# JarryChou/qcrypto-ldpc

Hardware: AMD Instinct MI355X
Metric: reconciled_key_Mbit_s (higher is better)
Workload: dtype f32

## Files before the change

### qcrypto-ldpc_amd/csrc/qldpc_engine.hip

```cpp
#include <hip/hip_runtime.h>

#include <algorithm>
#include <chrono>
#include <cstdio>
#include <cstdlib>
#include <cstring>
#include <new>
#include <optional>
#include <type_traits>
#include <vector>

#include "qldpc_engine_int.h"
#include "qldpc_kernels_edge.h"
#include "qldpc_kernels_chain.h"
#include "qldpc_kernels_compact.h"
#include "qldpc_kernels_fpost.h"
#include "qldpc_kernels_weakest.h"

extern "C" int qldpc_device_count(void)
{
    int n = 0;
    if (hipGetDeviceCount(&n) != hipSuccess) return 0;
    return n;
}
// ... 380 lines not shown
                if (code->max_dv < 32768) {
                    if ((rc = dev_alloc(d, &d->d_chain_order, (size_t)d->M)) || (rc = dev_alloc(d, &d->d_chain_dep, (size_t)d->E)) ||
                        (rc = dev_alloc(d, &d->d_chain_ver, (size_t)d->G * d->N)) || (rc = dev_alloc(d, &d->d_chain_ctl, QC_CTL_WORDS))) return rc;
                    HIPCHK(hipMemcpy(d->d_chain_order, chain_order.data(), sizeof(int) * (size_t)d->M, hipMemcpyHostToDevice));
                    HIPCHK(hipMemcpy(d->d_chain_dep, depv.data(), sizeof(int) * (size_t)d->E, hipMemcpyHostToDevice));
                    d->chain = 1;
                }
            }
        }
    }
    const size_t G = (size_t)d->G, FG = (size_t)d->FG;
    if (cfg->schedule == QLDPC_SCHED_FLOODING) {
        const size_t elems = d->msg_i8 ? (G * d->E * FG + 3) / 4 : (d->msg_half ? (G * d->E * FG + 1) / 2 : G * d->E * FG);
        if (d->msg_i8 && (rc = dev_alloc(d, &d->d_llr8, G * d->N * 64))) return rc;
        const char *coded_env = getenv("QLDPC_CODED_LLR");
        if (!(coded_env && coded_env[0] == '0') && (!d->msg_i8 || (coded_env && coded_env[0] == '1'))) {
            if ((rc = dev_alloc(d, &d->d_ybits, G * d->N * V))) return rc;
            if ((rc = dev_alloc(d, &d->d_fmag, G * FG))) return rc;
            if ((rc = dev_alloc(d, &d->d_fnch, G * FG))) return rc;
            if ((rc = dev_alloc(d, &d->d_vcls, ((size_t)d->N + 3) / 4 * 4))) return rc;
        }
        if ((rc = dev_alloc(d, &d->d_a, elems))) return rc;
        if ((rc = dev_alloc(d, &d->d_b, elems))) return rc;
        {
            bool ok = !d->msg_i8 && !d->msg_half && d->V == 1 && family_of(cfg->rule) == QK_FAM_MS && !cfg->enable_syndrome && code->max_dc <= QK_FP_DCMAX;
            for (auto &b : d->cn_buckets) ok = ok && b.cap > 0;
            if (const char *e = getenv("QLDPC_FLOOD_POST")) ok = ok && atoi(e) != 0;
            std::vector<uint32_t> tab;
            if (ok) { tab.resize((size_t)d->M); ok = qldpc_code_chain_table(code, tab.data()) == 1; }
            if (ok) {
                d->ira_K = code->ira_K;
                d->fp_vn = 1;
                if (const char *e = getenv("QLDPC_FLOOD_POST_VN")) d->fp_vn = atoi(e) != 0;
                if ((rc = make_buckets(d, code->vn_ptr, nullptr, d->ira_K, VN_CAPS, 2, d->fp_vn_buckets))) return rc;
                if (d->fp_vn) {
                    std::vector<int> vt((size_t)d->E);
                    for (int k = 0; k < d->E; k++) vt[(size_t)code->transpose[k]] = k;
                    if ((rc = make_fp_vn_classes(d, code->vn_ptr, d->ira_K, vt.data(), d->fp_vn_classes))) return rc;
                }
                if ((rc = dev_alloc(d, &d->d_fp_chain, (size_t)d->M))) return rc;
                HIPCHK(hipMemcpy(d->d_fp_chain, tab.data(), sizeof(uint32_t) * (size_t)d->M, hipMemcpyHostToDevice));
                const size_t post_n = G * d->N * 64, st_n = G * d->M * (64 * QK_FP_ROWS);
                float *base = d->d_a;
                if (post_n + 2 * st_n > elems) { if ((rc = dev_alloc(d, &d->d_fp_mem, post_n + 2 * st_n))) return rc; base = d->d_fp_mem; }
                d->fp_post = base; d->fp_st[0] = base + post_n; d->fp_st[1] = base + post_n + st_n;
                d->fpost = 1;
            }
        }
    } else if (d->msg_i8) {
        if ((rc = dev_alloc(d, &d->d_llr8, G * d->N * 64))) return rc;
        if ((rc = dev_alloc(d, &d->d_a, G * d->N * 64))) return rc;
        if ((rc = dev_alloc(d, &d->d_b, G * d->E * 64))) return rc;
    } else {
        if ((rc = dev_alloc(d, &d->d_a, G * d->N * FG))) return rc;
        if ((rc = dev_alloc(d, &d->d_b, G * d->E * FG))) return rc;
    }
    if ((rc = dev_alloc(d, &d->d_sgn, G * d->N * V))) return rc;
    if (d->msg_i8) d->d_hard = d->d_sgn;
    else if ((rc = dev_alloc(d, &d->d_hard, G * d->N * V))) return rc;
    if ((rc = dev_alloc(d, &d->d_unsat, G * V))) return rc;
    if ((rc = dev_alloc(d, &d->d_done, G * V))) return rc;
    if ((rc = dev_alloc(d, &d->d_depth, G * FG))) return rc;
    if ((rc = dev_alloc(d, &d->d_iters, G * FG))) return rc;
    d->gu.patience = cfg->giveup_patience;
    if (d->gu.patience > 0 && ((rc = dev_alloc(d, &d->gu.weight, G * FG)) || (rc = dev_alloc(d, &d->gu.last, G * FG)) || (rc = dev_alloc(d, &d->gu.best, G * FG)) ||
                               (rc = dev_alloc(d, &d->gu.since, G * FG)) || (rc = dev_alloc(d, &d->gu.gave, G * V)) || (rc = dev_alloc(d, &d->gu.total, 1)))) return rc;
// ... 116 lines not shown
    if (!d) return QLDPC_EINVAL;
    HIPCHK(hipSetDevice(d->device));
    HIPCHK(hipStreamSynchronize(d->stream));
    return QLDPC_OK;
}


struct prof_scope {
    qldpc_decoder *d; int kind; double bytes, moved; hipEvent_t a, b; bool on;
    prof_scope(qldpc_decoder *d_, int kind_, double bytes_, double moved_ = -1.0) : d(d_), kind(kind_), bytes(bytes_), moved(moved_ < 0.0 ? bytes_ : moved_), a(nullptr), b(nullptr), on(d_->prof_on != 0)
    {
        if (on) { (void)hipEventCreate(&a); (void)hipEventCreate(&b); (void)hipEventRecord(a, d->stream); }
    }
    ~prof_scope()
    {
        if (on) { (void)hipEventRecord(b, d->stream); d->prof_pending.push_back({kind, bytes, moved, a, b}); }
    }
};

extern "C" int qldpc_profile_enable(qldpc_decoder *d, int on) { if (!d) return QLDPC_EINVAL; d->prof_on = on; return QLDPC_OK; }

static int prof_fold(qldpc_decoder *d)
{
    if (d->prof_pending.empty()) return QLDPC_OK;
    HIPCHK(hipStreamSynchronize(d->stream));
    for (auto &r : d->prof_pending) {
        float ms = 0.0f;
        if (hipEventElapsedTime(&ms, r.a, r.b) == hipSuccess) {
            d->stats[r.kind].launches++;
            d->stats[r.kind].total_ms += ms;
            d->stats[r.kind].alg_bytes += r.bytes;
            d->stats[r.kind].moved_bytes += r.moved;
        }
        (void)hipEventDestroy(r.a); (void)hipEventDestroy(r.b);
    }
    d->prof_pending.clear();
    return QLDPC_OK;
}

extern "C" int qldpc_profile_read(qldpc_decoder *d, qldpc_kernel_stat *out, int cap)
{
    if (!d || (!out && cap > 0)) return QLDPC_EINVAL;
    HIPCHK(hipSetDevice(d->device));
    int rc = prof_fold(d);
    if (rc) return rc;
    int n = 0;
    for (int k = 0; k < KS_COUNT && n < cap; k++) if (d->stats[k].launches) out[n++] = d->stats[k];
    return n;
}

extern "C" int qldpc_profile_clear(qldpc_decoder *d)
{
    if (!d) return QLDPC_EINVAL;
    int rc = prof_fold(d);
    if (rc) return rc;
    for (int k = 0; k < KS_COUNT; k++) { d->stats[k].launches = 0; d->stats[k].total_ms = 0; d->stats[k].alg_bytes = 0; d->stats[k].moved_bytes = 0; }
    return QLDPC_OK;
}


static double msg_b(const qldpc_decoder *d) { return d->msg_i8 ? 1.0 : (d->msg_half ? 2.0 : 4.0); }
static double llr_b(const qldpc_decoder *d) { return d->msg_i8 ? 1.0 : 4.0; }
static double live_frames(const qldpc_decoder *d) { return (double)(d->live_lanes > 0 && d->live_lanes < d->n_frames ? d->live_lanes : d->n_frames); }
static double bytes_cn(const qldpc_decoder *d) { return 2.0 * d->E * msg_b(d) * live_frames(d); }
static double bytes_vn(const qldpc_decoder *d, int mode)
{
    if (mode != QK_VN_NORMAL) return ((double)d->E * msg_b(d) + d->N * llr_b(d)) * live_frames(d);
    return (2.0 * d->E * msg_b(d) + d->N * llr_b(d)) * live_frames(d);
}
// ... 26 lines not shown
template <int V, int MODE>
static int vn_pass(qldpc_decoder *d, float *post_out)
{
    prof_scope ps(d, KS_VN, bytes_vn(d, MODE), moved_vn(d, MODE));
    for (auto &b : d->vn_buckets) { qldpc_launch_vn<V, MODE>(d, b, post_out); LAUNCHCHK(); }
    return QLDPC_OK;
}
template <int V>
static int cn_pass(qldpc_decoder *d, bool first = false)
{
    prof_scope ps(d, KS_CN, bytes_cn(d), first && !d->msg_i8 ? ((double)d->E * msg_b(d) + d->N / 8.0) * live_frames(d) : -1.0);
    for (auto &b : d->cn_buckets) { qldpc_launch_cn<V>(d, b, first); LAUNCHCHK(); }
    d->remap_src = nullptr;
    return QLDPC_OK;
}
static double fp_info_edges(const qldpc_decoder *d) { return (double)d->E - (2.0 * d->M - 1.0); }
static double fp_chan(const qldpc_decoder *d, double vns) { return d->llr_coded ? vns / 8.0 : vns * 4.0; }
static double moved_cn_fpost(const qldpc_decoder *d, bool first)
{
    const double Ei = fp_info_edges(d), st = (double)QK_FP_ROWS * d->M * 4.0;
    if (first) return (Ei * 4.0 + st + fp_chan(d, d->N)) * live_frames(d);
    return (2.0 * Ei * 4.0 + 2.0 * st + fp_chan(d, d->M)) * live_frames(d);
}
static double moved_vn_fpost(const qldpc_decoder *d, bool rows_out, bool ballots)
{
    return (fp_info_edges(d) * 4.0 + fp_chan(d, d->ira_K) + (rows_out ? d->ira_K * 4.0 : 0.0) + (ballots ? d->ira_K / 4.0 : 0.0)) * live_frames(d);
}
static double fp_vn_rec_bytes(const qldpc_decoder *d)
{
    double b = 0.0;
    for (auto &c : d->fp_vn_classes) b += (double)c.n * QK_FPV_STRIDE(c.deg) * 4.0;
    return b * (live_frames(d) / 64.0);
}
static int cn_pass_fpost(qldpc_decoder *d, int ite)
{
    prof_scope ps(d, KS_CN, bytes_cn(d), moved_cn_fpost(d, ite == 0));
    for (auto &b : d->cn_buckets) { qldpc_launch_cn_fpost(d, b, ite); LAUNCHCHK(); }
    d->fp_last = ite & 1;
    return QLDPC_OK;
}
static int vn_pass_fpost(qldpc_decoder *d, float *post_out, bool between)
{
    const bool own = between && d->fp_vn;
    prof_scope ps(d, KS_VN, bytes_vn(d, QK_VN_POST), moved_vn_fpost(d, post_out != nullptr, !between) + (own ? fp_vn_rec_bytes(d) : 0.0));
    d->fp_between = between ? 1 : 0;
    if (own) { qldpc_launch_vn_fpost(d); LAUNCHCHK(); }
    for (auto &b : d->fp_vn_buckets)
        if (!own || b.cap == 0) { qldpc_launch_vn<1, QK_VN_POST>(d, b, post_out); LAUNCHCHK(); }
    d->fp_between = 0;
    return QLDPC_OK;
}
static int close_fpost(qldpc_decoder *d, float *post_out)
{
    const double b = ((double)QK_FP_ROWS * d->M * 4.0 + fp_chan(d, d->M) + (post_out ? d->M * 4.0 : 0.0) + d->M / 4.0) * live_frames(d);
    prof_scope ps(d, KS_VN, b, b);
    qldpc_launch_fpost_close(d, post_out);
    LAUNCHCHK();
    return QLDPC_OK;
}
static int run_flooding_post(qldpc_decoder *d)
{
    int rc;
    const int n_ite = d->cfg.n_ite;
    for (int ite = 0; ite < n_ite; ite++) {
        if ((rc = cn_pass_fpost(d, ite))) return rc;
        if (ite < n_ite - 1 && (rc = vn_pass_fpost(d, d->fp_post, true))) return rc;
    }
    d->last_iters = n_ite;
    if ((rc = vn_pass_fpost(d, nullptr, false))) return rc;
    return close_fpost(d, nullptr);
}

template <int V>
static int synd_pass(qldpc_decoder *d, const u64 *mask, int skip_done)
{
    prof_scope ps(d, KS_SYND, (double)d->E * 8.0 * d->G * V);
    const int g8 = (d->G + 7) / 8 * 8;
    const int Mp = (skip_done && d->M >= 4096) ? ((d->M / 8 + 255) / 256) * 256 : d->M;
    for (int part = 0; part < (Mp < d->M ? 2 : 1); part++) {
        const int lo = part ? Mp : 0, hi = part ? d->M : Mp;
        const int bx = std::max(1, std::min((hi - lo + 255) / 256, 4096 / std::max(1, d->G)));
        hipLaunchKernelGGL((qk_syndrome<V>), dim3((unsigned)((d->G < 8 ? d->G : g8) * bx)), dim3(256), 0, d->stream, mask, d->d_cn_var_t, d->max_dc, d->M, d->N,
                           d->d_unsat, d->d_done, skip_done, target_synd(d), d->G, bx, lo, hi, part);
    }
    LAUNCHCHK();
    return QLDPC_OK;
}
template <int V>
static int status_pass(qldpc_decoder *d, int ite_done)
{
    prof_scope ps(d, KS_STATUS, 0.0);
    hipLaunchKernelGGL((qk_status<V>), dim3((unsigned)d->G), dim3(64), 0, d->stream, d->d_unsat, d->d_done, d->d_depth, d->d_iters, d->G,
                       d->cfg.syndrome_depth, ite_done, d->d_active, d->d_work, (volatile int *)d->h_active_dev, ++d->poll_seq);
    LAUNCHCHK();
    return QLDPC_OK;
}
// ... 1094 lines not shown
    HIPCHK(hipSetDevice(d->device));
    return for_each_gen(d, [&](const int *origin, const u64 *fin, int n_slots) -> int {
        dim3 gs((unsigned)((n_slots + 255) / 256));
        with_v(d, [&](auto v) { hipLaunchKernelGGL((qk_giveup_out<v()>), gs, dim3(256), 0, d->stream, d->gu, d_gave, d_last_weight, d_best_weight, n_slots, origin, fin); });
        LAUNCHCHK();
        return (int)QLDPC_OK;
    });
}

extern "C" int qldpc_giveup_total(qldpc_decoder *d, uint64_t *frames)
{
    if (!d || !frames) return QLDPC_EINVAL;
    *frames = 0;
    if (d->gu.patience <= 0) return QLDPC_OK;
    HIPCHK(hipSetDevice(d->device));
    unsigned long long n = 0;
    HIPCHK(hipMemcpyAsync(&n, d->gu.total, sizeof(n), hipMemcpyDeviceToHost, d->stream));
    HIPCHK(hipStreamSynchronize(d->stream));
    *frames = n;
    return QLDPC_OK;
}

static int post_rows(qldpc_decoder *d, const char *who, const float **rows)
{
    int rc;
    if (d->cur_gen != 0) {
        qldpc_set_error("%s: the run compacted its active frames (%d times), the messages of frames that converged earlier are gone; "
                        "create the decoder with compact = 2 (or freeze_messages = 1) to read posteriors", who, d->compactions);
        return QLDPC_EUNSUPPORTED;
    }
    const float *src;
    if (d->cfg.schedule == QLDPC_SCHED_FLOODING) {
        if (!d->d_post) { if ((rc = dev_alloc(d, &d->d_post, (size_t)d->G * d->N * d->FG))) return rc; }
        if (d->fpost) { if ((rc = vn_pass_fpost(d, d->d_post, false)) || (rc = close_fpost(d, d->d_post))) return rc; }
        else if ((rc = with_v(d, [&](auto v) { return vn_pass<v(), QK_VN_POST>(d, d->d_post); }))) return rc;
        src = d->d_post;
    } else if (d->msg_i8) {
        if (!d->d_post) { if ((rc = dev_alloc(d, &d->d_post, (size_t)d->G * d->N * d->FG))) return rc; }
        const size_t n_dwords = (size_t)d->G * d->N * 64;
        hipLaunchKernelGGL(qi_post_to_f32, dim3((unsigned)std::min<size_t>((n_dwords + 255) / 256, 16384)), dim3(256), 0, d->stream, (const uint32_t *)d->d_a, d->d_post, n_dwords);
        LAUNCHCHK();
        src = d->d_post;
    } else {
        src = d->d_a;
    }
    *rows = src;
    return QLDPC_OK;
}

extern "C" int qldpc_fetch_post_dev(qldpc_decoder *d, float *d_post_out)
{
    if (!d || !d_post_out) return QLDPC_EINVAL;
    int rc = need_ran(d, "qldpc_fetch_post_dev");
    if (rc) return rc;
    HIPCHK(hipSetDevice(d->device));
    if (d->engine == QLDPC_ENGINE_EDGES) {
        return edge_vn<QK_VN_POST>(d, 0, 0, 1, d_post_out, -1);
    }
    const float *src;
    if ((rc = post_rows(d, "qldpc_fetch_post_dev", &src))) return rc;
    dim3 grid((unsigned)((d->N + 63) / 64), (unsigned)d->G);
    with_v(d, [&](auto v) { hipLaunchKernelGGL((qk_unload_f32<v()>), grid, dim3(256), 0, d->stream, src, d_post_out, d->N, d->n_frames); });
    LAUNCHCHK();
    return QLDPC_OK;
}

extern "C" int qldpc_fetch_weakest_dev(qldpc_decoder *d, const uint32_t *d_cand_bits, const int *d_take, int n_weak, uint32_t *d_weak_bits)
// ... 43 lines not shown
```

### qcrypto-ldpc_amd/csrc/qldpc_engine_int.h

```cpp
#ifndef QLDPC_ENGINE_INT_H
#define QLDPC_ENGINE_INT_H

#include <hip/hip_runtime.h>

#include <algorithm>
#include <vector>

#include "qldpc_hip.h"
#include "qldpc_kernels.h"
#include "qldpc_kernels_i8.h"
#include "qldpc_kernels_gang.h"
#include "qldpc_kernels_giveup.h"

enum { KS_CN = 0, KS_VN, KS_LAYER, KS_SYND, KS_STATUS, KS_LOAD, KS_FETCH, KS_VLAYER, KS_LAYER_REMAP, KS_COMPACT_ROWS, KS_LAYER_GANG, KS_COUNT };
static const char *const ks_names[KS_COUNT] = {"cn_update", "vn_update", "layer_update", "syndrome", "status", "load", "fetch", "vn_vlayer", "layer_update_remap", "compact_rows", "layer_update_gang"};

struct prof_rec { int kind; double bytes, moved; hipEvent_t a, b; };

struct bucket { int cap; int n; int *d_list; int *d_rec; };

struct fp_vn_class { int deg; int n; int *d_rec; };

struct gen_state {
    int G, cap;
    u64 *sgn, *hard, *unsat, *done, *ybits, *synd, *ebits;
    int *depth, *iters, *origin, *src;
    float *fmag; int *fnch;
    float *llr; uint32_t *llr8;
    int *gu_last, *gu_best, *gu_since; u64 *gu_gave;
    float *post, *msg;
};
#define QLDPC_MAX_GENS 6

struct qldpc_decoder {
    qldpc_decoder_cfg cfg;
    int N, M, E, K;
    int V, FG, G;
    int device;
    hipStream_t stream;
    int *d_cn_ptr, *d_cn_tr, *d_cn_var, *d_vn_ptr, *d_info_pos;
    int *d_vn_tr;
    int *d_cn_var_t, max_dc;
    std::vector<bucket> cn_buckets, vn_buckets;
    std::vector<std::vector<bucket>> layer_buckets;
    int n_layers;
    std::vector<bucket> vlayer_classes;
    int *d_vn_chk;
    double vl_rows;
    int layer_cst;
    int chain, chain_blocks, chain_lds; int *d_chain_order, *d_chain_dep, *d_chain_ver, *d_chain_ctl;
    qk_gang_entry *d_gang; std::vector<int> gang_off;
    int fpost, ira_K;
    std::vector<bucket> fp_vn_buckets;
    std::vector<fp_vn_class> fp_vn_classes;
    uint32_t *d_fp_chain;
    float *fp_post, *fp_st[2];
    float *d_fp_mem;
    int fp_last;
    int fp_between;
    int fp_vn;
    int layer_first;
    float *d_llr, *d_a, *d_b;
    float *d_post;
    u64 *d_sgn, *d_hard, *d_unsat, *d_done;
    int *d_depth, *d_iters, *d_active;
    int *h_active, *h_active_dev;
    int poll_seq;
    unsigned long long *d_work;
    qk_giveup gu;
    int G0;
    std::vector<gen_state> gens;
    int cur_gen, compact_mode, compactions;
    int live_lanes;
    float compact_ratio;
    const int *remap_src;
    const float *remap_msg;
    int *d_gcount, *d_goff;
    int llr_alt_cap[2]; float *d_llr_alt[2]; uint32_t *d_llr8_alt[2];
    int lay_alt_cap[2]; float *d_post_alt[2], *d_msg_alt[2];
    size_t bytes;
    int n_frames;
    int loaded, ran;
    int last_iters;
    int poll_every;
    u64 *d_synd;
    uint32_t *e_synd;
    int has_synd;
    float *h_in; int *h_out;
    int msg_half;
    u64 *d_ybits; float *d_fmag; int *d_fnch; uint8_t *d_vcls; int llr_coded;
    u64 *d_ebits; int has_erase;
    uint32_t *d_known; int has_known;
    int post_closes_run;
// ... 52 lines not shown
{
    if (mode == QK_VN_POST && d->fp_between) return 0;
    if (mode == QK_VN_POST) return 1 | (d->post_closes_run ? 2 : 0);
    return d->cfg.enable_syndrome ? 1 : 0;
}

struct gang_slot { int member, entry, n; };
struct gang_class { int cap, fam, cst; std::vector<gang_slot> slots; };
typedef std::vector<std::vector<gang_class>> gang_steps;
static inline void gang_plan_add(gang_steps &steps, int step, int cap, int fam, int cst, gang_slot s)
{
    if ((int)steps.size() <= step) steps.resize((size_t)step + 1);
    for (auto &c : steps[(size_t)step])
        if (c.cap == cap && c.fam == fam && c.cst == cst) { c.slots.push_back(s); return; }
    steps[(size_t)step].push_back(gang_class{cap, fam, cst, {s}});
}
struct qldpc_gang {
    std::vector<qldpc_decoder *> m;
    gang_steps steps;
    std::vector<int> buckets;
    int device;
    hipStream_t stream;
    long long stats[4];
};
int qldpc_launch_layer_gang(hipStream_t stream, int cap, int fam, int cst, const qk_gang_args &a, unsigned grid);

template <int V> void qldpc_launch_cn(qldpc_decoder *d, const bucket &b, bool first);
template <int V> void qldpc_launch_layer(qldpc_decoder *d, const bucket &b);
template <int V> void qldpc_launch_vlayer(qldpc_decoder *d, const bucket &b);
void qldpc_launch_layer_chain(qldpc_decoder *d, int sweep);
void qldpc_launch_cn_fpost(qldpc_decoder *d, const bucket &b, int ite);
void qldpc_launch_fpost_close(qldpc_decoder *d, float *post_out);
void qldpc_launch_vn_fpost(qldpc_decoder *d);
int qldpc_chain_resident_blocks(qldpc_decoder *d);
template <int V, int MODE> void qldpc_launch_vn(qldpc_decoder *d, const bucket &b, float *post_out);
#define QLDPC_DECLARE_LAUNCH(V)                                                                   \
    extern template void qldpc_launch_cn<V>(qldpc_decoder *, const bucket &, bool);                \
    extern template void qldpc_launch_layer<V>(qldpc_decoder *, const bucket &);                   \
    extern template void qldpc_launch_vlayer<V>(qldpc_decoder *, const bucket &);                  \
    extern template void qldpc_launch_vn<V, QK_VN_FIRST>(qldpc_decoder *, const bucket &, float *); \
    extern template void qldpc_launch_vn<V, QK_VN_NORMAL>(qldpc_decoder *, const bucket &, float *); \
    extern template void qldpc_launch_vn<V, QK_VN_POST>(qldpc_decoder *, const bucket &, float *);

#endif
```

### qcrypto-ldpc_amd/csrc/qldpc_kernels.h

```cpp
#ifndef QLDPC_KERNELS_H
#define QLDPC_KERNELS_H

#include <hip/hip_runtime.h>
#include <hip/hip_fp16.h>
#include <stdint.h>

typedef unsigned long long u64;

#ifndef QK_WAVES
#define QK_WAVES 4
#endif
#define QK_THREADS (QK_WAVES * 64)
#define QK_IDX_PAD 64

#define QK_FAM_MS 0
#define QK_REC_HDR 4
#define QK_FAM_SPA 1
#define QK_FAM_LSPA 2
#define QK_FAM_AMS 3

struct qk_rule {
    int rule;
    float param;
};
// ... 420 lines not shown
                for (int j = 0; j < V; j++) x[j] = qk_first_v2c(x[j], vin);
            } else if constexpr (REMAP) {
#pragma unroll
                for (int j = 0; j < V; j++) x[j] = qk_ldm1(vin_r[j] + (size_t)cn_tr[b + k] * FG);
            } else qk_load<V>(x, vin + (size_t)cn_tr[b + k] * FG);
#pragma unroll
            for (int j = 0; j < V; j++) qk_acc_in<FAM>(acc[j], qk_prep<FAM>(x[j]), rule);
        }
#pragma unroll
        for (int j = 0; j < V; j++) acc[j].finish(rule);
        for (int k = 0; k < deg; k++) {
            float x[V], o[V];
            const size_t off = (size_t)cn_tr[b + k] * FG;
            if constexpr (FIRST) {
                qk_coded_y<V>(x, coded, g, cn_var[b + k], N, lane, mg, nc);
#pragma unroll
                for (int j = 0; j < V; j++) x[j] = qk_first_v2c(x[j], vin);
            } else if constexpr (REMAP) {
#pragma unroll
                for (int j = 0; j < V; j++) x[j] = qk_ldm1(vin_r[j] + off);
            } else qk_load<V>(x, vin + off);
#pragma unroll
            for (int j = 0; j < V; j++) o[j] = acc[j].out(qk_prep<FAM>(x[j]), rule);
            qk_store_masked<V>(cout + (size_t)(b + k) * FG, o, frozen, any_frozen);
        }
    }
}


#define QK_VN_FIRST 0
#define QK_VN_NORMAL 1
#define QK_VN_POST 2

template <int V, int DVMAX, int UN, int MODE, typename MT, bool CODED = false>
__global__ __launch_bounds__(QK_THREADS) void qk_vn_flood(const MT *__restrict__ c2v, const float *__restrict__ llr,
                                                          MT *__restrict__ v2c, u64 *__restrict__ sgn, u64 *__restrict__ hard,
                                                          float *__restrict__ post_out,
                                                          const int *__restrict__ list, int n_list,
                                                          const int *__restrict__ vn_ptr, int N, size_t group_stride,
                                                          const u64 *__restrict__ done, qk_coded_llr coded = qk_coded_llr{}, int want_ballots = 1,
                                                          const int *__restrict__ vn_tr = nullptr)
{
    constexpr int FG = 64 * V;
    const int g = blockIdx.y;
    if ((MODE != QK_VN_POST || (want_ballots & 2)) && qk_group_done<V>(done, g)) return;
    const int lane = threadIdx.x & 63;
    const int wave = __builtin_amdgcn_readfirstlane(threadIdx.x >> 6);
    const MT *cin = c2v + (size_t)g * group_stride + lane * V;
    MT *vout = v2c + (size_t)g * group_stride + lane * V;
    const float *yin = llr + (size_t)g * N * FG + lane * V;
    const int i0 = (blockIdx.x * QK_WAVES + wave) * UN;
    if (i0 >= n_list) return;

    int vv[UN], bb[UN], dd[UN];
#pragma unroll
    for (int u = 0; u < UN; u++) {
        const int i = (i0 + u < n_list) ? i0 + u : i0;
        vv[u] = list[i];
    }
#pragma unroll
    for (int u = 0; u < UN; u++) { bb[u] = vn_ptr[vv[u]]; dd[u] = vn_ptr[vv[u] + 1] - bb[u]; }
    float y[UN][V], tmp[UN][V];
    auto channel = [&]() {
        if constexpr (CODED) {
            float mg[V];
            int nc[V];
#pragma unroll
            for (int j = 0; j < V; j++) { mg[j] = coded.fmag[(size_t)g * FG + lane * V + j]; nc[j] = coded.fnch[(size_t)g * FG + lane * V + j]; }
#pragma unroll
            for (int u = 0; u < UN; u++) qk_coded_y<V>(y[u], coded, g, vv[u], N, lane, mg, nc);
        } else {
#pragma unroll
            for (int u = 0; u < UN; u++) qk_ldm<V>(y[u], yin + (size_t)vv[u] * FG);
        }
    };
    if constexpr (MODE == QK_VN_FIRST || DVMAX <= 0) channel();

    if constexpr (MODE == QK_VN_FIRST) {
#pragma unroll
        for (int u = 0; u < UN; u++) {
            float o[V];
#pragma unroll
            for (int j = 0; j < V; j++) { tmp[u][j] = y[u][j] + 0.0f; o[j] = tmp[u][j] - 0.0f; }
            for (int k = 0; k < dd[u]; k++) qk_stm<V>(vout + (size_t)(bb[u] + k) * FG, o);
        }
    } else if constexpr (DVMAX > 0) {
        int tr[UN][DVMAX];
#pragma unroll
        for (int u = 0; u < UN; u++) {
#pragma unroll
            for (int k = 0; k < DVMAX; k++) tr[u][k] = vn_tr[bb[u] + k];
        }
        float m[UN][DVMAX][V];
#pragma unroll
        for (int u = 0; u < UN; u++) {
#pragma unroll
            for (int k = 0; k < DVMAX; k++)
                if (k < dd[u]) qk_ldm<V>(m[u][k], cin + (size_t)tr[u][k] * FG);
        }
        channel();
#pragma unroll
        for (int u = 0; u < UN; u++) {
            float sum[V];
#pragma unroll
            for (int j = 0; j < V; j++) sum[j] = 0.0f;
#pragma unroll
            for (int k = 0; k < DVMAX; k++)
                if (k < dd[u]) {
#pragma unroll
                    for (int j = 0; j < V; j++) sum[j] += m[u][k][j];
                }
#pragma unroll
            for (int j = 0; j < V; j++) tmp[u][j] = y[u][j] + sum[j];
            if constexpr (MODE == QK_VN_NORMAL) {
#pragma unroll
                for (int k = 0; k < DVMAX; k++)
                    if (k < dd[u]) {
                        float o[V];
#pragma unroll
                        for (int j = 0; j < V; j++) o[j] = tmp[u][j] - m[u][k][j];
                        qk_stm<V>(vout + (size_t)(bb[u] + k) * FG, o);
                    }
            }
        }
    } else {
#pragma unroll
        for (int u = 0; u < UN; u++) {
            float sum[V];
#pragma unroll
            for (int j = 0; j < V; j++) sum[j] = 0.0f;
            for (int k = 0; k < dd[u]; k++) {
                float m[V];
                qk_load<V>(m, cin + (size_t)vn_tr[bb[u] + k] * FG);
// ... 591 lines not shown
```

### qcrypto-ldpc_amd/csrc/qldpc_kernels_fpost.h

```cpp
#ifndef QLDPC_KERNELS_FPOST_H
#define QLDPC_KERNELS_FPOST_H

#include "qldpc_kernels.h"

#define QK_FP_ROWS 3
#define QK_FP_DCMAX 27
#define QK_FP_NONE 0xffu

__device__ __forceinline__ float qk_fp_msg(uint32_t w, int k, float c1, float c2)
{
    return qk_withsign(((int)(w >> 27) == k) ? c1 : c2, (w >> k) << 31);
}

template <int DCMAX, bool FIRST, bool CODED>
__global__ __launch_bounds__(QK_THREADS) void qk_cn_fpost(const float *__restrict__ post, const float *__restrict__ llr, float *__restrict__ c2v,
                                                          const float *st_in, float *st_out,
                                                          const int *__restrict__ list, int n_list,
                                                          const int *__restrict__ cn_ptr, const int *__restrict__ cn_var, const uint32_t *__restrict__ chain,
                                                          size_t group_stride, const u64 *__restrict__ done, qk_rule rule, const u64 *__restrict__ synd, int M, int N,
                                                          qk_coded_llr coded)
{
    static_assert(DCMAX > 0 && DCMAX <= QK_FP_DCMAX, "sign bits and the index share one word");
    const int g = blockIdx.y;
    const int lane = threadIdx.x & 63;
// ... 71 lines not shown
    }
    {
        const float own = qk_fp_msg(w, rp, c1, c2);
        const float sum0 = 0.0f + own;
        const float sum = (rnb != (int)QK_FP_NONE) ? sum0 + qk_fp_msg(rw, rnb & 31, rc1, rc2) : sum0;
        const float tmp = yr + sum;
        xr = tmp - own;
    }
    qk_acc<QK_FAM_MS> acc;
    acc.begin();
    if (synd) acc.sign = (uint32_t)((synd[(size_t)g * M + c] >> lane) & 1ull) << 31;
#pragma unroll
    for (int k = 0; k < DCMAX; k++)
        if (k < deg) {
            if (k == lpos) x[k] = xl;
            if (k == rpos) x[k] = xr;
            acc.in(x[k]);
        }
    acc.finish(rule);
    float *cout = c2v + (size_t)g * group_stride + lane;
    uint32_t nw = 0u, idx = 0u;
#pragma unroll
    for (int k = 0; k < DCMAX; k++)
        if (k < deg) {
            const float o = acc.out(x[k], rule);
            if (k != lpos && k != rpos) __builtin_nontemporal_store(o, cout + (size_t)(b + k) * 64);
            nw |= (qk_bits(o) >> 31) << k;
        }
#pragma unroll
    for (int k = DCMAX - 1; k >= 0; k--)
        if (k < deg) idx = (fabsf(x[k]) == acc.min1) ? (uint32_t)k : idx;
    float *so = st_out + srow;
    so[0] = acc.cst1; so[64] = acc.cst2; reinterpret_cast<uint32_t *>(so)[128] = nw | (idx << 27);
}

#define QK_FPV_DMAX 12
#define QK_FPV_CLASSES 4
#define QK_FPV_STRIDE(D) (((D) + 1 + 3) & ~3)
#define QK_FPV_UN(D) ((D) <= 4 ? 4 : 2)
struct qk_fpv_args {
    const int *rec[QK_FPV_CLASSES];
    int n[QK_FPV_CLASSES], deg[QK_FPV_CLASSES], blk_end[QK_FPV_CLASSES];
};
template <int D, int UN, bool CODED>
__device__ __forceinline__ void qk_vn_fpost_deg(const float *__restrict__ cin, const float *__restrict__ yin, float *__restrict__ pout,
                                                const int *__restrict__ rec, int n_list, int i0, int g, int lane, int N,
                                                const u64 *__restrict__ done, const qk_coded_llr &coded)
{
    constexpr int S = QK_FPV_STRIDE(D);
    if (i0 >= n_list) return;
    int w[UN][S];
#pragma unroll
    for (int u = 0; u < UN; u++) {
        const int i = (i0 + u < n_list) ? i0 + u : i0;
        const int4 *r = reinterpret_cast<const int4 *>(rec) + (size_t)i * (S / 4);
#pragma unroll
        for (int q = 0; q < S / 4; q++) {
            const int4 t = r[q];
            w[u][4 * q] = t.x; w[u][4 * q + 1] = t.y; w[u][4 * q + 2] = t.z; w[u][4 * q + 3] = t.w;
        }
    }
    if (qk_group_done<1>(done, g)) return;
    float m[UN][D > 0 ? D : 1];
#pragma unroll
    for (int u = 0; u < UN; u++) {
#pragma unroll
// ... 93 lines not shown
```

### qcrypto-ldpc_amd/csrc/qldpc_launch.hip

```cpp
#include "qldpc_engine_int.h"
#include "qldpc_kernels_h16.h"
#include "qldpc_kernels_cst.h"
#include "qldpc_kernels_vl.h"

#ifndef QL_V
#error "compile with -DQL_V=1, 2 or 4"
#endif

template <int V, int CAP, int FAM>
static void launch_cn_one(qldpc_decoder *d, const bucket &b, bool first)
{
    dim3 grid((unsigned)grid_x(b.n, 1), (unsigned)d->G);
    const qk_rule r = rule_of(d);
    if (first && !d->msg_i8) {
        const qk_coded_llr c = coded_llr_of(d);
        if (d->msg_half)
            hipLaunchKernelGGL((qk_cn_flood<V, CAP, FAM, __half, true>), grid, dim3(QK_THREADS), 0, d->stream, (const __half *)d->d_a, (__half *)d->d_b, b.d_list, b.n,
                               d->d_cn_ptr, d->d_cn_tr, (size_t)d->E * d->FG, d->d_done, r, d->freeze, target_synd(d), d->M, d->d_cn_var, d->N, c);
        else
            hipLaunchKernelGGL((qk_cn_flood<V, CAP, FAM, float, true>), grid, dim3(QK_THREADS), 0, d->stream, (const float *)d->d_a, d->d_b, b.d_list, b.n,
                               d->d_cn_ptr, d->d_cn_tr, (size_t)d->E * d->FG, d->d_done, r, d->freeze, target_synd(d), d->M, d->d_cn_var, d->N, c);
        return;
    }
    if (d->remap_src) {
// ... 153 lines not shown
                const qk_coded_llr c = coded_llr_of(d);
                hipLaunchKernelGGL((qi_vn_flood<CAP, UN, MODE, true>), grid, dim3(QK_THREADS), 0, d->stream, (const uint32_t *)d->d_b, (const uint32_t *)nullptr, (uint32_t *)d->d_a, d->d_sgn, (u64 *)nullptr,
                                   post_out, b.d_list, b.n, d->d_vn_ptr, d->N, (size_t)d->E * 64, d->d_done, c, d->quant_scale, want_ballots(d, MODE), d->d_vn_tr);
            } else
                hipLaunchKernelGGL((qi_vn_flood<CAP, UN, MODE, false>), grid, dim3(QK_THREADS), 0, d->stream, (const uint32_t *)d->d_b, d->d_llr8, (uint32_t *)d->d_a, d->d_sgn, (u64 *)nullptr,
                                   post_out, b.d_list, b.n, d->d_vn_ptr, d->N, (size_t)d->E * 64, d->d_done, qk_coded_llr{}, 0.0f, want_ballots(d, MODE), d->d_vn_tr);
        }
        return;
    }
    if (d->msg_half) launch_vn_k<V, CAP, UN, MODE, __half>(d, b, post_out);
    else launch_vn_k<V, CAP, UN, MODE, float>(d, b, post_out);
}
template <int V, int MODE>
void qldpc_launch_vn(qldpc_decoder *d, const bucket &b, float *post_out)
{
    if (MODE == QK_VN_FIRST) { launch_vn_one<V, 0, MODE>(d, b, post_out); return; }
    switch (b.cap) {
    case 4: launch_vn_one<V, 4, MODE>(d, b, post_out); break;
    case 12: launch_vn_one<V, 12, MODE>(d, b, post_out); break;
    default: launch_vn_one<V, 0, MODE>(d, b, post_out); break;
    }
}

template void qldpc_launch_cn<QL_V>(qldpc_decoder *, const bucket &, bool);
template void qldpc_launch_layer<QL_V>(qldpc_decoder *, const bucket &);
template void qldpc_launch_vlayer<QL_V>(qldpc_decoder *, const bucket &);
template void qldpc_launch_vn<QL_V, QK_VN_FIRST>(qldpc_decoder *, const bucket &, float *);
template void qldpc_launch_vn<QL_V, QK_VN_NORMAL>(qldpc_decoder *, const bucket &, float *);
template void qldpc_launch_vn<QL_V, QK_VN_POST>(qldpc_decoder *, const bucket &, float *);

#if QL_V == 1
#include "qldpc_kernels_fpost.h"

template <int DCMAX, bool FIRST>
static void launch_cn_fpost_one(qldpc_decoder *d, const bucket &b, int ite)
{
    dim3 grid((unsigned)grid_x(b.n, 1), (unsigned)d->G);
    const float *st_in = d->fp_st[(ite & 1) ^ 1];
    float *st_out = d->fp_st[ite & 1];
    if (d->llr_coded)
        hipLaunchKernelGGL((qk_cn_fpost<DCMAX, FIRST, true>), grid, dim3(QK_THREADS), 0, d->stream, (const float *)d->fp_post, (const float *)nullptr, d->d_b, st_in, st_out, b.d_list, b.n,
                           d->d_cn_ptr, d->d_cn_var, d->d_fp_chain, (size_t)d->E * 64, d->d_done, rule_of(d), target_synd(d), d->M, d->N, coded_llr_of(d));
    else
        hipLaunchKernelGGL((qk_cn_fpost<DCMAX, FIRST, false>), grid, dim3(QK_THREADS), 0, d->stream, (const float *)d->fp_post, (const float *)d->d_llr, d->d_b, st_in, st_out, b.d_list, b.n,
                           d->d_cn_ptr, d->d_cn_var, d->d_fp_chain, (size_t)d->E * 64, d->d_done, rule_of(d), target_synd(d), d->M, d->N, qk_coded_llr{});
}
void qldpc_launch_cn_fpost(qldpc_decoder *d, const bucket &b, int ite)
{
    switch (b.cap) {
    case 8: ite == 0 ? launch_cn_fpost_one<8, true>(d, b, ite) : launch_cn_fpost_one<8, false>(d, b, ite); break;
    case 12: ite == 0 ? launch_cn_fpost_one<12, true>(d, b, ite) : launch_cn_fpost_one<12, false>(d, b, ite); break;
    case 20: ite == 0 ? launch_cn_fpost_one<20, true>(d, b, ite) : launch_cn_fpost_one<20, false>(d, b, ite); break;
    default: ite == 0 ? launch_cn_fpost_one<QK_FP_DCMAX, true>(d, b, ite) : launch_cn_fpost_one<QK_FP_DCMAX, false>(d, b, ite); break;
    }
}
void qldpc_launch_vn_fpost(qldpc_decoder *d)
{
    const size_t nc = d->fp_vn_classes.size();
    for (size_t c0 = 0; c0 < nc; c0 += QK_FPV_CLASSES) {
        qk_fpv_args a{};
        int blocks = 0;
        for (size_t k = 0; k < QK_FPV_CLASSES; k++) {
            if (c0 + k < nc) {
                const fp_vn_class &c = d->fp_vn_classes[c0 + k];
                a.rec[k] = c.d_rec; a.n[k] = c.n; a.deg[k] = c.deg;
                blocks += grid_x(c.n, QK_FPV_UN(c.deg));
            }
            a.blk_end[k] = blocks;
        }
        dim3 grid((unsigned)blocks, (unsigned)d->G);
        if (d->llr_coded)
            hipLaunchKernelGGL((qk_vn_fpost<true>), grid, dim3(QK_THREADS), 0, d->stream, (const float *)d->d_b, (const float *)nullptr, d->fp_post, a,
                               d->N, (size_t)d->E * 64, d->d_done, coded_llr_of(d));
        else
            hipLaunchKernelGGL((qk_vn_fpost<false>), grid, dim3(QK_THREADS), 0, d->stream, (const float *)d->d_b, (const float *)d->d_llr, d->fp_post, a,
                               d->N, (size_t)d->E * 64, d->d_done, qk_coded_llr{});
    }
}
void qldpc_launch_fpost_close(qldpc_decoder *d, float *post_out)
{
    dim3 grid((unsigned)grid_x(d->M, 1), (unsigned)d->G);
    if (d->llr_coded)
        hipLaunchKernelGGL((qk_fpost_close<true>), grid, dim3(QK_THREADS), 0, d->stream, (const float *)d->fp_st[d->fp_last], (const float *)nullptr, d->d_fp_chain, d->d_sgn, d->d_hard, post_out,
                           d->M, d->N, d->ira_K, d->d_done, coded_llr_of(d));
    else
        hipLaunchKernelGGL((qk_fpost_close<false>), grid, dim3(QK_THREADS), 0, d->stream, (const float *)d->fp_st[d->fp_last], (const float *)d->d_llr, d->d_fp_chain, d->d_sgn, d->d_hard, post_out,
                           d->M, d->N, d->ira_K, d->d_done, qk_coded_llr{});
}

#include "qldpc_kernels_chain.h"

template <int DCMAX, int FAM>
static void launch_chain_one(qldpc_decoder *d, int sweep)
{
    const qk_rule r = rule_of(d);
    const int total = d->M * d->G;
    const unsigned grid = (unsigned)std::max(1, std::min((total + QK_WAVES - 1) / QK_WAVES, d->chain_blocks));
    hipLaunchKernelGGL((qk_cn_layer_chain<DCMAX, FAM>), dim3(grid), dim3(QK_THREADS), (size_t)d->chain_lds, d->stream, d->d_a, d->d_b, d->d_chain_order, d->M, d->G, d->d_cn_ptr, d->d_cn_var,
                       d->d_chain_dep, d->d_chain_ver, d->d_chain_ctl, sweep, d->N, (size_t)d->E * d->FG, d->d_done, r,
                       target_synd(d), d->layer_first, getenv("QLDPC_DEBUG") ? 1 : 0);
}
template <int FAM>
static void launch_chain_fam(qldpc_decoder *d, int sweep)
{
    if (d->max_dc <= 12) launch_chain_one<12, FAM>(d, sweep);
    else if (d->max_dc <= 20) launch_chain_one<20, FAM>(d, sweep);
    else launch_chain_one<40, FAM>(d, sweep);
}
void qldpc_launch_layer_chain(qldpc_decoder *d, int sweep)
{
    switch (family_of(d->cfg.rule)) {
    case QK_FAM_MS: launch_chain_fam<QK_FAM_MS>(d, sweep); break;
    case QK_FAM_SPA: launch_chain_fam<QK_FAM_SPA>(d, sweep); break;
    case QK_FAM_LSPA: launch_chain_fam<QK_FAM_LSPA>(d, sweep); break;
    default: launch_chain_fam<QK_FAM_AMS>(d, sweep); break;
    }
}
int qldpc_chain_resident_blocks(qldpc_decoder *d)
{
    int per_cu = 0, cus = 0;
// ... 14 lines not shown
```

Before: 2126.

## Batch groups in first flood-post CN pass and add scheduled final VN kernel

Adds a first-iteration check-node kernel that handles two to four frame groups per block. The code-structure loads (list, cn_ptr, cn_var, chain) are shared across those groups instead of being repeated per group. The final VN pass for degree-4 buckets now uses a variant with vectorised list loads and scheduling barriers that push memory loads ahead of use. Profiling scopes for the flood-post path are also reworked so consecutive kernels reuse a seam event instead of creating and recording two events each. The grouped kernel has fewer blocks and more registers per wave, which may reduce occupancy.

```diff
diff --git a/qcrypto-ldpc_amd/csrc/qldpc_engine.hip b/qcrypto-ldpc_amd/csrc/qldpc_engine.hip
--- a/qcrypto-ldpc_amd/csrc/qldpc_engine.hip
+++ b/qcrypto-ldpc_amd/csrc/qldpc_engine.hip
@@ -436,6 +436,12 @@
                 d->ira_K = code->ira_K;
                 d->fp_vn = 1;
                 if (const char *e = getenv("QLDPC_FLOOD_POST_VN")) d->fp_vn = atoi(e) != 0;
+                d->fp_first_groups = 4;
+                if (const char *e = getenv("QLDPC_FLOOD_POST_FIRST_GROUPS")) { const int x = atoi(e); if (x == 1 || x == 2 || x == 4) d->fp_first_groups = x; }
+                d->fp_close = 1;
+                if (const char *e = getenv("QLDPC_FLOOD_POST_CLOSE")) d->fp_close = atoi(e) != 0;
+                d->prof_markers = 0;
+                if (const char *e = getenv("QLDPC_PROF_MARKERS")) d->prof_markers = atoi(e) != 0;
                 if ((rc = make_buckets(d, code->vn_ptr, nullptr, d->ira_K, VN_CAPS, 2, d->fp_vn_buckets))) return rc;
                 if (d->fp_vn) {
                     std::vector<int> vt((size_t)d->E);
@@ -618,9 +624,10 @@
             d->stats[r.kind].alg_bytes += r.bytes;
             d->stats[r.kind].moved_bytes += r.moved;
         }
-        (void)hipEventDestroy(r.a); (void)hipEventDestroy(r.b);
-    }
+    }
+    for (auto &r : d->prof_pending) { if (!r.keep_a) (void)hipEventDestroy(r.a); (void)hipEventDestroy(r.b); }
     d->prof_pending.clear();
+    d->fp_seam = nullptr;
     return QLDPC_OK;
 }
 
@@ -713,9 +720,26 @@
     for (auto &c : d->fp_vn_classes) b += (double)c.n * QK_FPV_STRIDE(c.deg) * 4.0;
     return b * (live_frames(d) / 64.0);
 }
+struct fp_scope {
+    qldpc_decoder *d; int kind; double bytes, moved; hipEvent_t a; bool on, keep_a;
+    fp_scope(qldpc_decoder *d_, int kind_, double bytes_, double moved_) : d(d_), kind(kind_), bytes(bytes_), moved(moved_), a(nullptr), on(d_->prof_on != 0), keep_a(false)
+    {
+        if (!on) return;
+        if (!d->prof_markers && d->fp_seam) { a = d->fp_seam; keep_a = true; return; }
+        (void)hipEventCreate(&a); (void)hipEventRecord(a, d->stream);
+    }
+    ~fp_scope()
+    {
+        if (!on) return;
+        hipEvent_t b = nullptr;
+        (void)hipEventCreate(&b); (void)hipEventRecord(b, d->stream);
+        d->fp_seam = b;
+        d->prof_pending.push_back({kind, bytes, moved, a, b, keep_a});
+    }
+};
 static int cn_pass_fpost(qldpc_decoder *d, int ite)
 {
-    prof_scope ps(d, KS_CN, bytes_cn(d), moved_cn_fpost(d, ite == 0));
+    fp_scope ps(d, KS_CN, bytes_cn(d), moved_cn_fpost(d, ite == 0));
     for (auto &b : d->cn_buckets) { qldpc_launch_cn_fpost(d, b, ite); LAUNCHCHK(); }
     d->fp_last = ite & 1;
     return QLDPC_OK;
@@ -723,18 +747,22 @@
 static int vn_pass_fpost(qldpc_decoder *d, float *post_out, bool between)
 {
     const bool own = between && d->fp_vn;
-    prof_scope ps(d, KS_VN, bytes_vn(d, QK_VN_POST), moved_vn_fpost(d, post_out != nullptr, !between) + (own ? fp_vn_rec_bytes(d) : 0.0));
+    fp_scope ps(d, KS_VN, bytes_vn(d, QK_VN_POST), moved_vn_fpost(d, post_out != nullptr, !between) + (own ? fp_vn_rec_bytes(d) : 0.0));
     d->fp_between = between ? 1 : 0;
     if (own) { qldpc_launch_vn_fpost(d); LAUNCHCHK(); }
     for (auto &b : d->fp_vn_buckets)
-        if (!own || b.cap == 0) { qldpc_launch_vn<1, QK_VN_POST>(d, b, post_out); LAUNCHCHK(); }
+        if (!own || b.cap == 0) {
+            if (!between && b.cap == 4 && d->fp_close) qldpc_launch_vn_fpost_last(d, b, post_out);
+            else qldpc_launch_vn<1, QK_VN_POST>(d, b, post_out);
+            LAUNCHCHK();
+        }
     d->fp_between = 0;
     return QLDPC_OK;
 }
 static int close_fpost(qldpc_decoder *d, float *post_out)
 {
     const double b = ((double)QK_FP_ROWS * d->M * 4.0 + fp_chan(d, d->M) + (post_out ? d->M * 4.0 : 0.0) + d->M / 4.0) * live_frames(d);
-    prof_scope ps(d, KS_VN, b, b);
+    fp_scope ps(d, KS_VN, b, b);
     qldpc_launch_fpost_close(d, post_out);
     LAUNCHCHK();
     return QLDPC_OK;
@@ -743,6 +771,7 @@
 {
     int rc;
     const int n_ite = d->cfg.n_ite;
+    d->fp_seam = nullptr;
     for (int ite = 0; ite < n_ite; ite++) {
         if ((rc = cn_pass_fpost(d, ite))) return rc;
         if (ite < n_ite - 1 && (rc = vn_pass_fpost(d, d->fp_post, true))) return rc;
@@ -1903,7 +1932,7 @@
     const float *src;
     if (d->cfg.schedule == QLDPC_SCHED_FLOODING) {
         if (!d->d_post) { if ((rc = dev_alloc(d, &d->d_post, (size_t)d->G * d->N * d->FG))) return rc; }
-        if (d->fpost) { if ((rc = vn_pass_fpost(d, d->d_post, false)) || (rc = close_fpost(d, d->d_post))) return rc; }
+        if (d->fpost) { d->fp_seam = nullptr; if ((rc = vn_pass_fpost(d, d->d_post, false)) || (rc = close_fpost(d, d->d_post))) return rc; }
         else if ((rc = with_v(d, [&](auto v) { return vn_pass<v(), QK_VN_POST>(d, d->d_post); }))) return rc;
         src = d->d_post;
     } else if (d->msg_i8) {
diff --git a/qcrypto-ldpc_amd/csrc/qldpc_engine_int.h b/qcrypto-ldpc_amd/csrc/qldpc_engine_int.h
--- a/qcrypto-ldpc_amd/csrc/qldpc_engine_int.h
+++ b/qcrypto-ldpc_amd/csrc/qldpc_engine_int.h
@@ -15,7 +15,7 @@
 enum { KS_CN = 0, KS_VN, KS_LAYER, KS_SYND, KS_STATUS, KS_LOAD, KS_FETCH, KS_VLAYER, KS_LAYER_REMAP, KS_COMPACT_ROWS, KS_LAYER_GANG, KS_COUNT };
 static const char *const ks_names[KS_COUNT] = {"cn_update", "vn_update", "layer_update", "syndrome", "status", "load", "fetch", "vn_vlayer", "layer_update_remap", "compact_rows", "layer_update_gang"};
 
-struct prof_rec { int kind; double bytes, moved; hipEvent_t a, b; };
+struct prof_rec { int kind; double bytes, moved; hipEvent_t a, b; bool keep_a; };
 
 struct bucket { int cap; int n; int *d_list; int *d_rec; };
 
@@ -59,6 +59,10 @@
     int fp_last;
     int fp_between;
     int fp_vn;
+    int fp_first_groups;
+    int fp_close;
+    int prof_markers;
+    hipEvent_t fp_seam;
     int layer_first;
     float *d_llr, *d_a, *d_b;
     float *d_post;
@@ -177,6 +181,7 @@
 void qldpc_launch_cn_fpost(qldpc_decoder *d, const bucket &b, int ite);
 void qldpc_launch_fpost_close(qldpc_decoder *d, float *post_out);
 void qldpc_launch_vn_fpost(qldpc_decoder *d);
+void qldpc_launch_vn_fpost_last(qldpc_decoder *d, const bucket &b, float *post_out);
 int qldpc_chain_resident_blocks(qldpc_decoder *d);
 template <int V, int MODE> void qldpc_launch_vn(qldpc_decoder *d, const bucket &b, float *post_out);
 #define QLDPC_DECLARE_LAUNCH(V)                                                                   \
diff --git a/qcrypto-ldpc_amd/csrc/qldpc_kernels.h b/qcrypto-ldpc_amd/csrc/qldpc_kernels.h
--- a/qcrypto-ldpc_amd/csrc/qldpc_kernels.h
+++ b/qcrypto-ldpc_amd/csrc/qldpc_kernels.h
@@ -476,7 +476,7 @@
 #define QK_VN_NORMAL 1
 #define QK_VN_POST 2
 
-template <int V, int DVMAX, int UN, int MODE, typename MT, bool CODED = false>
+template <int V, int DVMAX, int UN, int MODE, typename MT, bool CODED = false, bool AHEAD = false>
 __global__ __launch_bounds__(QK_THREADS) void qk_vn_flood(const MT *__restrict__ c2v, const float *__restrict__ llr,
                                                           MT *__restrict__ v2c, u64 *__restrict__ sgn, u64 *__restrict__ hard,
                                                           float *__restrict__ post_out,
@@ -497,13 +497,29 @@
     if (i0 >= n_list) return;
 
     int vv[UN], bb[UN], dd[UN];
-#pragma unroll
-    for (int u = 0; u < UN; u++) {
-        const int i = (i0 + u < n_list) ? i0 + u : i0;
-        vv[u] = list[i];
-    }
-#pragma unroll
-    for (int u = 0; u < UN; u++) { bb[u] = vn_ptr[vv[u]]; dd[u] = vn_ptr[vv[u] + 1] - bb[u]; }
+    bool whole = false;
+    if constexpr (AHEAD) {
+        typedef int qk_ivec __attribute__((ext_vector_type(UN)));
+        whole = i0 + UN <= n_list;
+        if (whole) {
+            const qk_ivec t = *reinterpret_cast<const qk_ivec *>(list + i0);
+#pragma unroll
+            for (int u = 0; u < UN; u++) vv[u] = t[u];
+        }
+    }
+    if (!whole) {
+#pragma unroll
+        for (int u = 0; u < UN; u++) {
+            const int i = (i0 + u < n_list) ? i0 + u : i0;
+            vv[u] = list[i];
+        }
+    }
+    if constexpr (AHEAD) __builtin_amdgcn_sched_barrier(0);
+#pragma unroll
+    for (int u = 0; u < UN; u++) { bb[u] = vn_ptr[vv[u]]; dd[u] = vn_ptr[vv[u] + 1]; }
+    if constexpr (AHEAD) __builtin_amdgcn_sched_barrier(0);
+#pragma unroll
+    for (int u = 0; u < UN; u++) dd[u] -= bb[u];
     float y[UN][V], tmp[UN][V];
     auto channel = [&]() {
         if constexpr (CODED) {
@@ -535,6 +551,13 @@
 #pragma unroll
             for (int k = 0; k < DVMAX; k++) tr[u][k] = vn_tr[bb[u] + k];
         }
+        if constexpr (AHEAD) {
+#pragma unroll
+            for (int u = 0; u < UN; u++) {
+#pragma unroll
+                for (int k = 0; k < DVMAX; k++) asm volatile("" ::"s"(tr[u][k]));
+            }
+        }
         float m[UN][DVMAX][V];
 #pragma unroll
         for (int u = 0; u < UN; u++) {
@@ -543,6 +566,16 @@
                 if (k < dd[u]) qk_ldm<V>(m[u][k], cin + (size_t)tr[u][k] * FG);
         }
         channel();
+        if constexpr (AHEAD) {
+#pragma unroll
+            for (int u = 0; u < UN; u++) {
+#pragma unroll
+                for (int k = 0; k < DVMAX; k++) {
+#pragma unroll
+                    for (int j = 0; j < V; j++) asm volatile("" : "+v"(m[u][k][j]));
+                }
+            }
+        }
 #pragma unroll
         for (int u = 0; u < UN; u++) {
             float sum[V];
diff --git a/qcrypto-ldpc_amd/csrc/qldpc_kernels_fpost.h b/qcrypto-ldpc_amd/csrc/qldpc_kernels_fpost.h
--- a/qcrypto-ldpc_amd/csrc/qldpc_kernels_fpost.h
+++ b/qcrypto-ldpc_amd/csrc/qldpc_kernels_fpost.h
@@ -127,6 +127,102 @@
         if (k < deg) idx = (fabsf(x[k]) == acc.min1) ? (uint32_t)k : idx;
     float *so = st_out + srow;
     so[0] = acc.cst1; so[64] = acc.cst2; reinterpret_cast<uint32_t *>(so)[128] = nw | (idx << 27);
+}
+
+template <int DCMAX, bool CODED, int GW>
+__global__ __launch_bounds__(QK_THREADS) void qk_cn_fpost_first(const float *__restrict__ llr, float *__restrict__ c2v, float *__restrict__ st_out,
+                                                                const int *__restrict__ list, int n_list,
+                                                                const int *__restrict__ cn_ptr, const int *__restrict__ cn_var, const uint32_t *__restrict__ chain,
+                                                                size_t group_stride, const u64 *__restrict__ done, qk_rule rule, const u64 *__restrict__ synd, int M, int N, int G,
+                                                                qk_coded_llr coded)
+{
+    static_assert(DCMAX > 0 && DCMAX <= QK_FP_DCMAX, "sign bits and the index share one word");
+    static_assert(GW > 1 && GW <= 4, "a run of two to four groups");
+    const int g0 = blockIdx.y * GW;
+    const int lane = threadIdx.x & 63;
+    const int wave = __builtin_amdgcn_readfirstlane(threadIdx.x >> 6);
+    const int i = blockIdx.x * QK_WAVES + wave;
+    if (i >= n_list) return;
+    int gg[GW];
+    float mg[GW];
+    int nc[GW];
+    u64 dn[GW], sy[GW];
+#pragma unroll
+    for (int j = 0; j < GW; j++) {
+        gg[j] = (g0 + j < G) ? g0 + j : G - 1;
+        mg[j] = 0.0f; nc[j] = 0;
+        if constexpr (CODED) { mg[j] = coded.fmag[(size_t)gg[j] * 64 + lane]; nc[j] = coded.fnch[(size_t)gg[j] * 64 + lane]; }
+        dn[j] = done[gg[j]];
+    }
+    const int c = list[i];
+    const int b = cn_ptr[c];
+    const int deg = cn_ptr[c + 1] - b;
+    const uint32_t ch = chain[c];
+    const int lpos = (int)(ch & 0xffu), rpos = (int)((ch >> 8) & 0xffu);
+#pragma unroll
+    for (int j = 0; j < GW; j++) sy[j] = synd ? synd[(size_t)gg[j] * M + c] : 0ull;
+    int vid[DCMAX];
+    qk_coded_w wl[GW];
+    float y[CODED ? 1 : GW][DCMAX];
+    if constexpr (CODED) {
+        const int kl = lane < deg ? lane : (deg > 0 ? deg - 1 : 0);
+        const int vlane = cn_var[b + kl];
+        const uint32_t cls = (reinterpret_cast<const uint32_t *>(coded.vcls)[vlane >> 2] >> ((vlane & 3) * 8)) & 0xffu;
+        const u64 *eb = coded.ebits ? coded.ebits : coded.ybits;
+        const u64 em = coded.ebits ? ~0ull : 0ull;
+#pragma unroll
+        for (int j = 0; j < GW; j++) {
+            const size_t at = (size_t)gg[j] * N + vlane;
+            wl[j].cls = cls; wl[j].yb = coded.ybits[at]; wl[j].eb = eb[at] & em;
+        }
+#pragma unroll
+        for (int j = 0; j < GW; j++) { asm volatile("" ::"v"(wl[j].yb), "v"(wl[j].eb)); qk_pin_lane(mg[j], nc[j]); }
+#pragma unroll
+        for (int k = 0; k < DCMAX; k++) vid[k] = __builtin_amdgcn_readlane(vlane, k);
+    } else {
+#pragma unroll
+        for (int k = 0; k < DCMAX; k++) vid[k] = cn_var[b + k];
+#pragma unroll
+        for (int j = 0; j < GW; j++) {
+            const float *yin = llr + (size_t)gg[j] * N * 64 + lane;
+#pragma unroll
+            for (int k = 0; k < DCMAX; k++) y[j][k] = (k < deg) ? yin[(size_t)vid[k] * 64] : 0.0f;
+        }
+    }
+#pragma unroll
+    for (int j = 0; j < GW; j++) {
+        if (g0 + j >= G || dn[j] == ~0ull) continue;
+        const int g = g0 + j;
+        float x[DCMAX];
+#pragma unroll
+        for (int k = 0; k < DCMAX; k++) {
+            float yk;
+            if constexpr (CODED) yk = qk_coded_y_of(qk_coded_w_of_lane(wl[j], k), vid[k], mg[j], nc[j]);
+            else yk = y[j][k];
+            x[k] = qk_first_v2c(yk, (const float *)nullptr);
+        }
+        qk_acc<QK_FAM_MS> acc;
+        acc.begin();
+        if (synd) acc.sign = (uint32_t)((sy[j] >> lane) & 1ull) << 31;
+#pragma unroll
+        for (int k = 0; k < DCMAX; k++)
+            if (k < deg) acc.in(x[k]);
+        acc.finish(rule);
+        float *cout = c2v + (size_t)g * group_stride + lane;
+        uint32_t nw = 0u, idx = 0u;
+#pragma unroll
+        for (int k = 0; k < DCMAX; k++)
+            if (k < deg) {
+                const float o = acc.out(x[k], rule);
+                if (k != lpos && k != rpos) __builtin_nontemporal_store(o, cout + (size_t)(b + k) * 64);
+                nw |= (qk_bits(o) >> 31) << k;
+            }
+#pragma unroll
+        for (int k = DCMAX - 1; k >= 0; k--)
+            if (k < deg) idx = (fabsf(x[k]) == acc.min1) ? (uint32_t)k : idx;
+        float *so = st_out + ((size_t)g * M + c) * (64 * QK_FP_ROWS) + lane;
+        so[0] = acc.cst1; so[64] = acc.cst2; reinterpret_cast<uint32_t *>(so)[128] = nw | (idx << 27);
+    }
 }
 
 #define QK_FPV_DMAX 12
diff --git a/qcrypto-ldpc_amd/csrc/qldpc_launch.hip b/qcrypto-ldpc_amd/csrc/qldpc_launch.hip
--- a/qcrypto-ldpc_amd/csrc/qldpc_launch.hip
+++ b/qcrypto-ldpc_amd/csrc/qldpc_launch.hip
@@ -209,9 +209,24 @@
 #if QL_V == 1
 #include "qldpc_kernels_fpost.h"
 
+template <int DCMAX, int GW>
+static void launch_cn_fpost_first(qldpc_decoder *d, const bucket &b)
+{
+    dim3 grid((unsigned)grid_x(b.n, 1), (unsigned)((d->G + GW - 1) / GW));
+    if (d->llr_coded)
+        hipLaunchKernelGGL((qk_cn_fpost_first<DCMAX, true, GW>), grid, dim3(QK_THREADS), 0, d->stream, (const float *)nullptr, d->d_b, d->fp_st[0], b.d_list, b.n,
+                           d->d_cn_ptr, d->d_cn_var, d->d_fp_chain, (size_t)d->E * 64, d->d_done, rule_of(d), target_synd(d), d->M, d->N, d->G, coded_llr_of(d));
+    else
+        hipLaunchKernelGGL((qk_cn_fpost_first<DCMAX, false, GW>), grid, dim3(QK_THREADS), 0, d->stream, (const float *)d->d_llr, d->d_b, d->fp_st[0], b.d_list, b.n,
+                           d->d_cn_ptr, d->d_cn_var, d->d_fp_chain, (size_t)d->E * 64, d->d_done, rule_of(d), target_synd(d), d->M, d->N, d->G, qk_coded_llr{});
+}
 template <int DCMAX, bool FIRST>
 static void launch_cn_fpost_one(qldpc_decoder *d, const bucket &b, int ite)
 {
+    if constexpr (FIRST) {
+        if (d->fp_first_groups == 2) { launch_cn_fpost_first<DCMAX, 2>(d, b); return; }
+        if (d->fp_first_groups == 4) { launch_cn_fpost_first<DCMAX, 4>(d, b); return; }
+    }
     dim3 grid((unsigned)grid_x(b.n, 1), (unsigned)d->G);
     const float *st_in = d->fp_st[(ite & 1) ^ 1];
     float *st_out = d->fp_st[ite & 1];
@@ -263,6 +278,17 @@
     else
         hipLaunchKernelGGL((qk_fpost_close<false>), grid, dim3(QK_THREADS), 0, d->stream, (const float *)d->fp_st[d->fp_last], (const float *)d->d_llr, d->d_fp_chain, d->d_sgn, d->d_hard, post_out,
                            d->M, d->N, d->ira_K, d->d_done, qk_coded_llr{});
+}
+void qldpc_launch_vn_fpost_last(qldpc_decoder *d, const bucket &b, float *post_out)
+{
+    constexpr int UN = 8;
+    dim3 grid((unsigned)grid_x(b.n, UN), (unsigned)d->G);
+    if (d->llr_coded)
+        hipLaunchKernelGGL((qk_vn_flood<1, 4, UN, QK_VN_POST, float, true, true>), grid, dim3(QK_THREADS), 0, d->stream, (const float *)d->d_b, (const float *)nullptr, d->d_a, d->d_sgn, d->d_hard,
+                           post_out, b.d_list, b.n, d->d_vn_ptr, d->N, (size_t)d->E * d->FG, d->d_done, coded_llr_of(d), want_ballots(d, QK_VN_POST), d->d_vn_tr);
+    else
+        hipLaunchKernelGGL((qk_vn_flood<1, 4, UN, QK_VN_POST, float, false, true>), grid, dim3(QK_THREADS), 0, d->stream, (const float *)d->d_b, d->d_llr, d->d_a, d->d_sgn, d->d_hard,
+                           post_out, b.d_list, b.n, d->d_vn_ptr, d->N, (size_t)d->E * d->FG, d->d_done, qk_coded_llr{}, want_ballots(d, QK_VN_POST), d->d_vn_tr);
 }
 
 #include "qldpc_kernels_chain.h"
```

After: 2141 (median of 6 runs). Within noise of the previous version (+0.7%).
